# wangxb29/PPST

Measured on AMD Instinct MI355X. Metric: 512x512 portrait swaps/sec/GPU, higher is better.
Workload: dtype bf16x3 (fp32 split into hi+lo bf16, 3 MFMA passes, fp32 accumulate); 1 GPU; simple_swapping 512x512 batch=8 per GPU, generator+encoders forward only (BASELINE configs[1]); image_parallel=1 batch per rank, no data-path collective

## Files before the change

### include/ppst_hip.h

```cpp
#ifndef PPST_HIP_H
#define PPST_HIP_H

#include <stddef.h>
#include <stdint.h>

#ifdef __cplusplus
extern "C" {
#endif

#define PPST_OK 0
#define PPST_EINVAL (-1)
#define PPST_EUNSUPPORTED (-2)
#define PPST_ENULL (-3)

enum { PPST_F32 = 0, PPST_F16 = 1, PPST_BF16 = 2, PPST_F64 = 3  };

enum { PPST_PAD_ZERO = 0, PPST_PAD_REFLECT = 1, PPST_PAD_REPLICATE = 2 };

enum { PPST_ACT_NONE = 0, PPST_ACT_LRELU = 1 , PPST_ACT_PRELU = 2 };

#define PPST_ABI_VERSION 3
int ppst_version(void);

#define PPST_ST_F32 0
// ... 87 lines not shown
  int32_t out_h, out_w, out_ld, cout;
  int32_t nsteps, n_groups;
  int32_t pad_mode;
  int32_t in_off_y, in_off_x;
  int32_t out_sy, out_sx;
  int32_t act;
  int32_t precision;
  int32_t res_ld;
  int32_t tile_h, tile_w;
  int32_t halo;
  int32_t bn;
  const void* in_scale_shift;
  const void* in_prelu;
  int32_t in_c, in_act;
  int32_t flop_steps;
  int32_t tile_rows;
  int32_t a_slots;
  int32_t early_a;
  int32_t variant;
  int32_t reserved0;
  int32_t dual_b;
  int32_t io_st;
  int32_t k64;
  const void* in_res;
  int32_t in_res_ld;
  int32_t ksplit;
  const int32_t* ksplit_starts;
  void* ksplit_scratch;
  unsigned* ksplit_flags;
  uint32_t ksplit_epoch;
} ppst_conv_args;

int ppst_conv2d_mfma(const ppst_conv_args* a, void* stream);
int64_t ppst_conv_pack_wino_bytes(int cout, int cin);
int ppst_conv_pack_wino(const void* w, int64_t sn, int64_t sc, int64_t sy, int64_t sx, float scale, int cout, int cin,
                        void* out, void* stream);
int ppst_conv2d_f32(const ppst_conv_args* a, const void* w, int64_t sn, int64_t sc, int64_t sy, int64_t sx, float wscale,
                    const int32_t* src_c, const int32_t* src_ky, const int32_t* src_kx, void* stream);
int ppst_conv_tiles(int tile_h, int tile_w, int tile_rows);

int ppst_conv1x1_small_cin(const void* x, const void* w, const void* bias, void* y,
                           int64_t npix, int cin, int in_ld, int cout, float wscale,
                           int act, void* stream);
int ppst_conv1x1_small_cin_st(const void* x, const void* w, const void* bias, void* y,
                              int64_t npix, int cin, int in_ld, int cout, float wscale,
                              int act, int y_st , void* stream);
int ppst_conv1x1_small_cout(const void* x, const void* w, const void* bias, void* y,
                            int64_t npix, int cin, int cout, float wscale, void* stream);
int ppst_conv1x1_small_cout_st(const void* x, const void* w, const void* bias, void* y,
                               int64_t npix, int cin, int cout, float wscale, int x_st , void* stream);
int ppst_torgb_apply_st(const void* x, const void* scale_shift, const void* res, int res_ld, float out_scale, const void* w,
                        const void* bias, void* y, int B, int H, int W, int cin, float wscale, int x_st, void* stream);

int ppst_in_stats(const void* x, void* partial, int B, int H, int W, int C, int ld,
                  int rep_pad, int* n_partials, void* stream);
int ppst_in_finalize(const void* partial, int n_partials, const void* style,
                     int style_ld ,
                     const void* post_bias ,
                     void* scale_shift , int B, int C, double count,
                     float eps, void* stream);
int ppst_affine_act(const void* x, const void* scale_shift, const void* res,
                    const void* res_scale_shift , void* y,
                    int B, int64_t hw, int C, int x_ld, int res_ld, int y_ld,
                    int act , const void* prelu,
                    float out_scale,
                    int res_up2_w ,
// ... 328 lines not shown
```

### ppst_amd/_lib.py

```python
import ctypes
import os

import torch

HERE = os.path.dirname(os.path.abspath(__file__))
LIB_PATH = os.environ.get("PPST_HIP_LIB") or os.path.join(HERE, "libppst_hip.so")

if not os.path.exists(LIB_PATH):
    raise ImportError(
        "ppst_amd: %s is missing -- build it with `python -m ppst_amd.build` "
        "(hipcc --offload-arch=gfx950). There is no CPU fallback." % LIB_PATH)

lib = ctypes.CDLL(LIB_PATH)

vp, i32, i64, f32, f64 = ctypes.c_void_p, ctypes.c_int, ctypes.c_int64, ctypes.c_float, ctypes.c_double


class PackJob(ctypes.Structure):
    _fields_ = [("w", vp), ("sn", i64), ("sc", i64), ("sy", i64), ("sx", i64), ("src_c", vp), ("src_ky", vp), ("src_kx", vp),
                ("out", vp), ("total", i64), ("block0", i64), ("scale", f32), ("cout", i32), ("bn", i32), ("nsteps", i32),
                ("n_groups", i32), ("x3", i32), ("f16", i32), ("nblocks", i32), ("dual", i32)]


class UpscaleJob(ctypes.Structure):
# ... 47 lines not shown
        ("nsteps", i32), ("n_groups", i32), ("pad_mode", i32),
        ("in_off_y", i32), ("in_off_x", i32), ("out_sy", i32), ("out_sx", i32),
        ("act", i32), ("precision", i32), ("res_ld", i32), ("tile_h", i32), ("tile_w", i32),
        ("halo", i32), ("bn", i32), ("in_scale_shift", vp), ("in_prelu", vp), ("in_c", i32), ("in_act", i32),
        ("flop_steps", i32), ("tile_rows", i32), ("a_slots", i32), ("early_a", i32), ("variant", i32), ("reserved0", i32), ("dual_b", i32), ("io_st", i32), ("k64", i32),
        ("in_res", vp), ("in_res_ld", i32), ("ksplit", i32), ("ksplit_starts", vp),
        ("ksplit_scratch", vp), ("ksplit_flags", vp), ("ksplit_epoch", ctypes.c_uint32),
    ]


_SIGS = {
    "ppst_version": (i32, []),
    "ppst_guided_filter_tune": (i32, [i32, i32]),
    "ppst_upfirdn2d": (i32, [vp, vp, vp] + [i32] * 14 + [i32, vp]),
    "ppst_blur_nhwc": (i32, [vp, vp, vp] + [i32] * 10 + [vp, i32, vp]),
    "ppst_blur_nhwc_st": (i32, [vp, vp, vp] + [i32] * 10 + [vp, i32, i32, vp]),
    "ppst_fused_bias_act": (i32, [vp, vp, vp, vp, i64, i32, i32, i32, i32, f32, f32, i32, vp]),
    "ppst_nchw_to_nhwc": (i32, [vp, vp, i32, i32, i32, i32, vp]),
    "ppst_nhwc_to_nchw": (i32, [vp, vp, i32, i32, i32, i32, vp]),
    "ppst_conv_pack": (i32, [vp, i64, i64, i64, i64, f32, i32, i32, vp, vp, vp, i32, i32, i32, vp, vp]),
    "ppst_conv_pack_k64": (i32, [vp, i64, i64, i64, i64, f32, i32, i32, vp, vp, vp, i32, i32, i32, i32, vp, vp]),
    "ppst_conv_pack_up9_bytes": (i64, [i32, i32]),
    "ppst_conv_pack_up9": (i32, [vp, i64, i64, i64, i64, f32, i32, i32, vp, vp]),
    "ppst_conv_pack_wino_bytes": (i64, [i32, i32]),
    "ppst_conv_pack_wino": (i32, [vp, i64, i64, i64, i64, f32, i32, i32, vp, vp]),
    "ppst_conv_pack_dual": (i32, [vp, i64, i64, i64, i64, f32, i32, vp, vp, vp, i32, i32, i32, vp, vp]),
    "ppst_upscale_weight": (i32, [vp, vp, i32, i32, f32, vp]),
    "ppst_dgrad_s2d_stack_weight": (i32, [vp, vp, i32, i32, vp]),
    "ppst_depth_to_space_st": (i32, [vp, vp, i32, i32, i32, i32, i32, i32, i32, vp]),
    "ppst_pack_job_blocks": (i32, [i64]),
    "ppst_conv_pack_batch": (i32, [vp, i32, i32, vp]),
    "ppst_upscale_weight_batch": (i32, [vp, i32, i32, vp]),
    "ppst_conv2d_mfma": (i32, [ctypes.POINTER(ConvArgs), vp]),
    "ppst_conv2d_f32": (i32, [ctypes.POINTER(ConvArgs), vp, i64, i64, i64, i64, f32, vp, vp, vp, vp]),
    "ppst_conv_tiles": (i32, [i32, i32, i32]),
    "ppst_conv1x1_small_cin": (i32, [vp, vp, vp, vp, i64, i32, i32, i32, f32, i32, vp]),
    "ppst_conv1x1_small_cin_st": (i32, [vp, vp, vp, vp, i64, i32, i32, i32, f32, i32, i32, vp]),
    "ppst_conv1x1_small_cout": (i32, [vp, vp, vp, vp, i64, i32, i32, f32, vp]),
    "ppst_conv1x1_small_cout_st": (i32, [vp, vp, vp, vp, i64, i32, i32, f32, i32, vp]),
    "ppst_torgb_apply_st": (i32, [vp, vp, vp, i32, f32, vp, vp, vp, i32, i32, i32, i32, f32, i32, vp]),
    "ppst_in_stats": (i32, [vp, vp, i32, i32, i32, i32, i32, i32, ctypes.POINTER(i32), vp]),
    "ppst_in_finalize": (i32, [vp, i32, vp, i32, vp, vp, i32, i32, f64, f32, vp]),
    "ppst_affine_act": (i32, [vp, vp, vp, vp, vp, i32, i64, i32, i32, i32, i32, i32, vp, f32, i32, vp]),
    "ppst_affine_act_st": (i32, [vp, vp, vp, vp, vp, i32, i64, i32, i32, i32, i32, i32, vp, f32, i32, i32, i32, vp]),
    "ppst_affine_act_stats": (i32, [vp, vp, vp, vp, vp, vp, i32, i32, i32, i32, i32, i32, i32, i32, vp, f32, i32, i32, vp]),
    "ppst_upsample_nearest2": (i32, [vp, vp, i32, i32, i32, i32, vp]),
    "ppst_upsample_nearest2_st": (i32, [vp, vp, i32, i32, i32, i32, i32, vp]),
    "ppst_gap_gmp_ws": (i64, [i32, i64, i32]),
    "ppst_gap_gmp": (i32, [vp, vp, vp, vp, i32, i32, i32, i32, i32, vp]),
    "ppst_gap_gmp_st": (i32, [vp, vp, vp, vp, i32, i32, i32, i32, i32, i32, vp]),
    "ppst_avgpool": (i32, [vp, vp, i32, i32, i32, i32, i32, i32, i32, vp]),
    "ppst_bilinear": (i32, [vp, vp, i32, i32, i32, i32, i32, i32, i32, i32, vp]),
    "ppst_head_tail": (i32, [vp, vp, vp, vp, vp] + [i32] * 10 + [vp]),
    "ppst_maxpool2": (i32, [vp, vp, i32, i32, i32, i32, vp]),
    "ppst_linear": (i32, [vp, vp, vp, vp, i32, i32, i32, f32, f32, i32, i32, vp]),
    "ppst_l2norm_rows": (i32, [vp, vp, i32, i32, f32, i32, vp]),
    "ppst_lerp": (i32, [vp, vp, vp, i64, f32, vp]),
    "ppst_linear_grouped": (i32, [vp, i32, vp]),
    "ppst_l2norm_rows_grouped": (i32, [vp, i32, vp]),
    "ppst_lerp_grouped": (i32, [vp, i32, vp]),
    "ppst_gap_gmp_multi_level_ws": (i64, [vp, i32, i32]),
    "ppst_gap_gmp_multi_level": (i32, [vp, i32, i32, vp, i32, vp]),
    "ppst_spatial_modulation": (i32, [vp, vp, vp, vp, i32, i64, i32, vp]),
    "ppst_spatial_modulation_st": (i32, [vp, vp, vp, vp, i32, i64, i32, i32, vp]),
    "ppst_rselfcorr": (i32, [vp, vp, i32, i32, i32, i32, i32, vp]),
    "ppst_corr_prep": (i32, [vp, vp, i32, i32, i32, i32, vp]),
# ... 150 lines not shown
```

### ppst_amd/csrc/conv1x1.hip

```cpp
#include "conv_common.h"

struct C1Args {
  const float* x;
  const unsigned char* wpack;
  const int4* steps;
  float* y;
  const float* bias;
  const float* noise;
  const float* prelu;
  float* stats;
  const float* residual;
  float noise_weight, out_scale;
  int B, hw, in_ld, out_ld, cout, nsteps, act, res_ld, n_tiles, tiles;
  int in_h, in_w, out_h, out_w, tiles_x, pad_mode;
  const float* in_ss;
  const float* in_prelu;
  int in_c, in_act;
  const float* in_res;
  int in_res_ld;
};

#define C1_GROUP 8
#define C1_BLOB 8192

// ... 91 lines not shown
  };
  CONV_EPI_DISPATCH(SPEC, epi_passes, act, resm);
  if (a.stats) {
#pragma unroll
    for (int nt = 0; nt < NT; ++nt) {
      float4 u = s1[nt], w = s2[nt];
      float* uv[8] = {&u.x, &u.y, &u.z, &u.w, &w.x, &w.y, &w.z, &w.w};
#pragma unroll
      for (int q = 0; q < 8; ++q) {
        float t = *uv[q];
        t += __builtin_bit_cast(float, __builtin_amdgcn_mov_dpp(__builtin_bit_cast(int, t), 0xB1, 0xf, 0xf, true));
        t += __builtin_bit_cast(float, __builtin_amdgcn_mov_dpp(__builtin_bit_cast(int, t), 0x4E, 0xf, 0xf, true));
        t += __builtin_bit_cast(float, __builtin_amdgcn_mov_dpp(__builtin_bit_cast(int, t), 0x141, 0xf, 0xf, true));
        t += __builtin_bit_cast(float, __builtin_amdgcn_mov_dpp(__builtin_bit_cast(int, t), 0x140, 0xf, 0xf, true));
        *uv[q] = t;
      }
      if (r16 == 0) conv_epi_put_sums(&red[wave][nt * 16 + g * 4][0], u, w);
    }
    __syncthreads();
    if (tid < (NT > 4 ? 128 : 64)) {
      const int n = ntile * (NT > 4 ? 128 : 64) + tid;
      if (n < a.cout) {
        float t0 = 0.f, t1 = 0.f;
#pragma unroll
        for (int wv = 0; wv < 8; ++wv) { t0 += red[wv][tid][0]; t1 += red[wv][tid][1]; }
        float* o = a.stats + (((int64_t)b * a.tiles + mblk) * a.cout + n) * 2;
        o[0] = t0;
        o[1] = t1;
      }
    }
  }
}

template <int INSS, bool TAPS = false, int NT_ = 4, int PREC = 0, int IOS = PPST_ST_F32>
__global__ __launch_bounds__(512, 4) void conv1x1_stream_kernel(C1Args a) {
  constexpr int MT = 2, NT = NT_;
  constexpr bool X3 = PREC == 0;
  static_assert(IOS == PPST_ST_F32 || IOS == (PREC == 3 ? PPST_ST_F16 : PREC == 1 ? PPST_ST_BF16 : -1), "half storage: single-pass modes");
  constexpr int ES = IOS == PPST_ST_F32 ? 4 : 2;
  constexpr int BLOB1 = X3 ? C1_BLOB : C1_BLOB / 2;
  __shared__ uint4 sB[C1_GROUP * BLOB1 / 16];
  __shared__ float red[8][64][2];

  const int wid = xcd_block_id(blockIdx.x, gridDim.x);
  const int ntile = wid % a.n_tiles;
  int mblk = wid / a.n_tiles;
  const int b = mblk / a.tiles;
  mblk -= b * a.tiles;
  const int tid = threadIdx.x, lane = tid & 63, wave = __builtin_amdgcn_readfirstlane(tid >> 6);
  const int r16 = lane & 15, g = lane >> 4;
  const int pbase = mblk * 256 + wave * 32;
  const int tyi = TAPS ? mblk / a.tiles_x : 0, txi = TAPS ? mblk - tyi * a.tiles_x : 0;
  const int oy0 = tyi * 16 + wave * 2, ox = txi * 16 + r16;
  const unsigned char* xb = (const unsigned char*)a.x + (int64_t)b * (TAPS ? a.in_h * a.in_w : a.hw) * a.in_ld * ES;
  const unsigned char* wblob = a.wpack + (int64_t)ntile * a.nsteps * BLOB1;
#if defined(__HIP_DEVICE_COMPILE__)
  typedef const __attribute__((address_space(4))) int4* StepPtr;
#else
  typedef const int4* StepPtr;
#endif
  StepPtr steps = (StepPtr)a.steps;

  int64_t aoff[MT];
  bool pok[MT];
#pragma unroll
  for (int mt = 0; mt < MT; ++mt) {
    const int p = pbase + mt * 16 + r16;
    pok[mt] = TAPS ? true : p < a.hw;
    aoff[mt] = TAPS ? 0 : (int64_t)(pok[mt] ? p : 0) * a.in_ld + g * 8;
  }
  const float in_slope = (INSS && a.in_act == PPST_ACT_PRELU && a.in_prelu) ? a.in_prelu[0] : 0.f;
  auto in_act = [&](float t) -> float { return conv_in_act(t, a.in_act, in_slope); };

  f32x4 acc[MT][NT];
#pragma unroll
  for (int i = 0; i < MT; ++i)
#pragma unroll
    for (int j = 0; j < NT; ++j) acc[i][j] = (f32x4){0.f, 0.f, 0.f, 0.f};

  float4 raw[MT][2], ss[4];
  float4 rres[INSS == 2 ? MT : 1][2];
  auto a_load = [&](int4 d) {
    const int chan = d.x;
// ... 1 lines not shown
      int ix = ox + d.z;
      bool xok = ix >= 0 && ix < a.in_w;
      ix = conv_pad_index(ix, a.in_w, a.pad_mode);
#pragma unroll
      for (int mt = 0; mt < MT; ++mt) {
        int iy = oy0 + mt + d.y;
        const bool yok = iy >= 0 && iy < a.in_h;
        iy = conv_pad_index(iy, a.in_h, a.pad_mode);
        pok[mt] = a.pad_mode != PPST_PAD_ZERO || (xok && yok);
        aoff[mt] = ((int64_t)iy * a.in_w + ix) * a.in_ld + g * 8;
      }
    }
#pragma unroll
    for (int mt = 0; mt < MT; ++mt) {
      const float4* p = (const float4*)(xb + (aoff[mt] + chan) * ES);
      raw[mt][0] = p[0];
      if (IOS == PPST_ST_F32) raw[mt][1] = p[1];
      if (INSS == 2) {
        const int pp = pbase + mt * 16 + r16;
        const float4* q = (const float4*)(a.in_res + ((int64_t)b * a.hw + (pok[mt] ? pp : 0)) * a.in_res_ld + g * 8 + chan);
        rres[mt][0] = q[0];
        rres[mt][1] = q[1];
      }
    }
    if (INSS) {
      const float4* q = (const float4*)(a.in_ss + ((int64_t)b * a.in_c + chan + g * 8) * 2);
      ss[0] = q[0]; ss[1] = q[1]; ss[2] = q[2]; ss[3] = q[3];
    }
  };
  a_load(steps[0]);

  for (int s0 = 0; s0 < a.nsteps; s0 += C1_GROUP) {
    const int ng = a.nsteps - s0 < C1_GROUP ? a.nsteps - s0 : C1_GROUP;
    if (s0) __syncthreads();
    for (int i = tid; i < ng * (BLOB1 / 16); i += 512) sB[i] = ((const uint4*)(wblob + (int64_t)s0 * BLOB1))[i];
    __syncthreads();
    for (int sl = 0; sl < ng; ++sl) {
      const int s = s0 + sl;
      bf16x8 ah[MT], al[MT];
      bool vok[MT];
#pragma unroll
      for (int mt = 0; mt < MT; ++mt) vok[mt] = pok[mt];
#pragma unroll
      for (int mt = 0; mt < MT; ++mt) {
        if (IOS != PPST_ST_F32 && !INSS) {
          const float4 z = vok[mt] ? raw[mt][0] : make_float4(0.f, 0.f, 0.f, 0.f);
          ah[mt] = __builtin_bit_cast(bf16x8, z);
          al[mt] = ah[mt];
          continue;
        }
        float v[8] = {raw[mt][0].x, raw[mt][0].y, raw[mt][0].z, raw[mt][0].w, raw[mt][1].x, raw[mt][1].y, raw[mt][1].z, raw[mt][1].w};
        if (IOS != PPST_ST_F32) c1_unpack8<IOS>(raw[mt][0], v);
        if (INSS) {
          const float sc[8] = {ss[0].x, ss[0].z, ss[1].x, ss[1].z, ss[2].x, ss[2].z, ss[3].x, ss[3].z};
          const float sh[8] = {ss[0].y, ss[0].w, ss[1].y, ss[1].w, ss[2].y, ss[2].w, ss[3].y, ss[3].w};
#pragma unroll
          for (int j = 0; j < 8; ++j) {
            float t = sc[j] * v[j] + sh[j];
            if (INSS == 2) {
              const float4 r4 = rres[mt][j >> 2];
              t += (j & 3) == 0 ? r4.x : (j & 3) == 1 ? r4.y : (j & 3) == 2 ? r4.z : r4.w;
            }
            v[j] = in_act(t);
          }
        }
#pragma unroll
        for (int j = 0; j < 8; ++j)
          if (!vok[mt]) v[j] = 0.f;
        c1_cvt8<PREC>(v, ah[mt], al[mt]);
      }
      if (s + 1 < a.nsteps) a_load(steps[s + 1]);
      const unsigned char* bs = (const unsigned char*)sB + sl * BLOB1 + g * 1024 + r16 * 16;
#pragma unroll
      for (int nt = 0; nt < NT; ++nt) {
        const bf16x8 bh = *(const bf16x8*)(bs + nt * 256);
        bf16x8 bl = bh;
        if (X3) bl = *(const bf16x8*)(bs + nt * 256 + 4096);
#pragma unroll
        for (int mt = 0; mt < MT; ++mt) acc[mt][nt] = c1_mfma<PREC>(bh, bl, ah[mt], al[mt], acc[mt][nt]);
      }
    }
  }

  c1_epilogue<MT, NT, TAPS, X3, IOS>(a, acc, red, b, mblk, ntile, pbase, oy0, ox, tid, wave, r16, g);
}

#define C3_GROUP 9
template <int CTRL>
__device__ __forceinline__ bf16x8 c3_shift(bf16x8 edge, bf16x8 centre) {
  typedef int __attribute__((ext_vector_type(4))) i4;
  const i4 e = __builtin_bit_cast(i4, edge), c = __builtin_bit_cast(i4, centre);
  i4 r;
#pragma unroll
  for (int i = 0; i < 4; ++i) r[i] = __builtin_amdgcn_update_dpp(e[i], c[i], CTRL, 0xf, 0xf, false);
  return __builtin_bit_cast(bf16x8, r);
}

template <bool INSS, int NT_, int PREC = 0, int IOS = PPST_ST_F32>
__global__ __launch_bounds__(512, NT_ > 4 ? 2 : 4) void conv3x3_direct_kernel(C1Args a) {
  constexpr int MT = 2, NT = NT_;
  constexpr bool X3 = PREC == 0;
  static_assert(IOS == PPST_ST_F32 || IOS == (PREC == 3 ? PPST_ST_F16 : PREC == 1 ? PPST_ST_BF16 : -1), "half storage: single-pass modes");
  constexpr int ES = IOS == PPST_ST_F32 ? 4 : 2;
  constexpr int PSTR = (NT > 4 ? 128 : 64) * 16;
  constexpr int BLOB = (X3 ? 8 : 4) * PSTR;
  __shared__ uint4 sB[C3_GROUP * BLOB / 16];
  __shared__ float red[8][NT > 4 ? 128 : 64][2];
  const int tid = threadIdx.x, lane = tid & 63, wave = __builtin_amdgcn_readfirstlane(tid >> 6);
  const int r16 = lane & 15, g = lane >> 4;
  const int total = a.B * a.tiles * a.n_tiles;
  const int per = (total + (int)gridDim.x - 1) / (int)gridDim.x;
  const int w_beg = blockIdx.x * per, w_end = w_beg + per < total ? w_beg + per : total;
  const int nchunks = a.nsteps / 9;
  const bool keep_b = nchunks == 1 && a.n_tiles == 1;
  for (int wid = w_beg; wid < w_end; ++wid) {
  const int ntile = wid % a.n_tiles;
  int mblk = wid / a.n_tiles;
// ... 75 lines not shown
#pragma unroll
    for (int r = 0; r < 4; ++r) {
      bf16x8 ch, cl, eh, el;
      convert(rawc, okc, ch, cl);
      convert(rawe, oke, eh, el);
      if (r < 3) row_load(chan, r + 1);
      else if (c + 1 < nchunks) { ss_load(chan_next); row_load(chan_next, 0); }
#pragma unroll
      for (int dxi = 0; dxi < 3; ++dxi) {
        const bf16x8 fh = dxi == 0 ? c3_shift<0x111>(eh, ch) : (dxi == 1 ? ch : c3_shift<0x101>(eh, ch));
        const bf16x8 fl = dxi == 0 ? c3_shift<0x111>(el, cl) : (dxi == 1 ? cl : c3_shift<0x101>(el, cl));
#pragma unroll
        for (int mt = 0; mt < MT; ++mt) {
          const int dyi = r - mt;
          if (dyi < 0 || dyi > 2) continue;
          const unsigned char* bs = (const unsigned char*)sB + (dyi * 3 + dxi) * BLOB + g * PSTR + r16 * 16;
#pragma unroll
          for (int nt = 0; nt < NT; ++nt) {
            const bf16x8 bh = *(const bf16x8*)(bs + nt * 256);
            bf16x8 bl = bh;
            if (X3) bl = *(const bf16x8*)(bs + nt * 256 + 4 * PSTR);
            acc[mt][nt] = c1_mfma<PREC>(bh, bl, fh, fl, acc[mt][nt]);
          }
        }
        __builtin_amdgcn_sched_barrier(0);
      }
    }
    chan = chan_next;
  }
  c1_epilogue<MT, NT, true, (X3 && NT <= 4), IOS>(a, acc, red, b, mblk, ntile, 0, oy0, ox, tid, wave, r16, g);
  }
}

static inline int64_t blocks_of(const ppst_conv_args* a, int tiles, int n_tiles) { return (int64_t)a->B * tiles * n_tiles; }
int ppst_conv1x1_stream_launch(const ppst_conv_args* a, int n_tiles, int tiles, hipStream_t st) {
  C1Args k;
  k.x = (const float*)a->x; k.wpack = (const unsigned char*)a->wpack; k.steps = (const int4*)a->steps; k.y = (float*)a->y;
  k.bias = (const float*)a->bias; k.noise = (const float*)a->noise; k.prelu = (const float*)a->prelu;
  k.stats = (float*)a->stats; k.residual = (const float*)a->residual;
  k.noise_weight = a->noise_weight; k.out_scale = a->out_scale;
  k.B = a->B; k.hw = a->out_h * a->out_w; k.in_ld = a->in_ld; k.out_ld = a->out_ld; k.cout = a->cout; k.nsteps = a->nsteps;
  k.act = a->act; k.res_ld = a->res_ld; k.n_tiles = n_tiles; k.tiles = tiles;
  k.in_ss = (const float*)a->in_scale_shift; k.in_prelu = (const float*)a->in_prelu; k.in_c = a->in_c; k.in_act = a->in_act;
  k.in_res = (const float*)a->in_res; k.in_res_ld = a->in_res_ld;
  if ((int64_t)tiles * 256 < k.hw) return PPST_EINVAL;
  if (k.in_res) {
    PPST_LAUNCH((conv1x1_stream_kernel<2, false, 4, 0, PPST_ST_F32>), dim3((unsigned)blocks_of(a, tiles, n_tiles)), dim3(512), 0, st, k);
    return PPST_LAUNCH_CHECK();
  }
  const int64_t blocks = (int64_t)a->B * tiles * n_tiles;
  if (blocks > 0x7fffffff) return PPST_EINVAL;
#define LS(PREC_, IOS_)                                                                                               \
  do {                                                                                                                \
    if (k.in_ss) PPST_LAUNCH((conv1x1_stream_kernel<1, false, 4, PREC_, IOS_>), dim3((unsigned)blocks), dim3(512), 0, st, k);   \
    else PPST_LAUNCH((conv1x1_stream_kernel<0, false, 4, PREC_, IOS_>), dim3((unsigned)blocks), dim3(512), 0, st, k);          \
  } while (0)
  if (a->precision == 1) { if (a->io_st) LS(1, PPST_ST_BF16); else LS(1, PPST_ST_F32); }
  else if (a->precision == 3) { if (a->io_st) LS(3, PPST_ST_F16); else LS(3, PPST_ST_F32); }
  else LS(0, PPST_ST_F32);
#undef LS
  return PPST_LAUNCH_CHECK();
}

int ppst_conv_direct_launch(const ppst_conv_args* a, int n_tiles, int tiles_y, int tiles_x, hipStream_t st) {
  C1Args k;
  k.x = (const float*)a->x; k.wpack = (const unsigned char*)a->wpack; k.steps = (const int4*)a->steps; k.y = (float*)a->y;
  k.bias = (const float*)a->bias; k.noise = (const float*)a->noise; k.prelu = (const float*)a->prelu;
  k.stats = (float*)a->stats; k.residual = (const float*)a->residual;
  k.noise_weight = a->noise_weight; k.out_scale = a->out_scale;
  k.B = a->B; k.hw = a->out_h * a->out_w; k.in_ld = a->in_ld; k.out_ld = a->out_ld; k.cout = a->cout; k.nsteps = a->nsteps;
  k.act = a->act; k.res_ld = a->res_ld; k.n_tiles = n_tiles; k.tiles = tiles_y * tiles_x;
  k.in_ss = (const float*)a->in_scale_shift; k.in_prelu = (const float*)a->in_prelu; k.in_c = a->in_c; k.in_act = a->in_act;
  k.in_h = a->in_h; k.in_w = a->in_w; k.out_h = a->out_h; k.out_w = a->out_w; k.tiles_x = tiles_x; k.pad_mode = a->pad_mode;
  const int64_t blocks = (int64_t)a->B * k.tiles * n_tiles;
  if (blocks > 0x7fffffff) return PPST_EINVAL;
  const bool nt2 = a->cout <= 32;
#define LD(INSS_, PREC_, IOS_)                                                                                       \
  do {                                                                                                               \
    if (nt2) PPST_LAUNCH((conv1x1_stream_kernel<INSS_, true, 2, PREC_, IOS_>), dim3((unsigned)blocks), dim3(512), 0, st, k);       \
    else PPST_LAUNCH((conv1x1_stream_kernel<INSS_, true, 4, PREC_, IOS_>), dim3((unsigned)blocks), dim3(512), 0, st, k);           \
  } while (0)
#define LDP(PREC_, IOS_) do { if (k.in_ss) LD(1, PREC_, IOS_); else LD(0, PREC_, IOS_); } while (0)
  if (a->precision == 1) { if (a->io_st) LDP(1, PPST_ST_BF16); else LDP(1, PPST_ST_F32); }
  else if (a->precision == 3) { if (a->io_st) LDP(3, PPST_ST_F16); else LDP(3, PPST_ST_F32); }
  else LDP(0, PPST_ST_F32);
#undef LDP
#undef LD
  return PPST_LAUNCH_CHECK();
}

int ppst_conv3x3_direct_launch(const ppst_conv_args* a, int n_tiles, int tiles_y, int tiles_x, hipStream_t st) {
  if (a->nsteps % 9) return PPST_EINVAL;
  C1Args k;
// ... 28 lines not shown
```

### ppst_amd/csrc/conv_mfma.hip

```cpp
#include "conv_common.h"


#ifdef PPST_CONV_CLOCK
__device__ unsigned long long* g_clock_buf = nullptr;
__device__ int g_clock_n = 1;
extern "C" int ppst_conv_clock_buffer(void* buf, int n) {
  if (n <= 0) return PPST_EINVAL;
  if (hipMemcpyToSymbol(HIP_SYMBOL(g_clock_buf), &buf, sizeof(buf)) != hipSuccess) return PPST_EINVAL;
  return hipMemcpyToSymbol(HIP_SYMBOL(g_clock_n), &n, sizeof(n)) == hipSuccess ? PPST_OK : PPST_EINVAL;
}
#endif
typedef _Float16 __attribute__((ext_vector_type(8))) half8;
__device__ __forceinline__ unsigned short f2h(float f) { return __builtin_bit_cast(unsigned short, (_Float16)f); }
template <int WM, int WN, int HALO, bool X3, bool INSS, int NAS = 0, bool F16 = false, int IOS = PPST_ST_F32>
__global__ __launch_bounds__(64 * WM * WN, NAS ? 2 : 1) void conv_mfma_kernel(ConvKArgs a) {
  static_assert(IOS == PPST_ST_F32 || (!X3 && IOS == (F16 ? PPST_ST_F16 : PPST_ST_BF16)), "half storage: single-pass modes");
  constexpr int ES = IOS == PPST_ST_F32 ? 4 : 2;
  constexpr int NT = 64 * WM * WN;
  constexpr int TH = 4 * WM, TW = 16;
  constexpr int HH = TH + 2 * HALO, HW = TW + 2 * HALO, HP = HH * HW;
  constexpr int PLANE = (WM == 2) ? HP * 16 : ((HP * 16 + 255) / 256) * 256;
  constexpr int NPL = X3 ? 8 : 4;
  constexpr int NPLB = X3 ? 8 : 4;
  constexpr int ABUF = NPL * PLANE;
// ... 621 lines not shown
extern "C" int ppst_prof_enable(int on) {
  g_prof_on = on;
  g_ev_used = 0;
  if (on) g_prof_dropped = 0;
  return PPST_OK;
}
extern "C" int ppst_prof_collect(double* ms, int64_t* launches, double* flop) {
  double t = 0.0, f = 0.0;
  for (int i = 0; i < g_ev_used; ++i) {
    float e = 0.f;
    hipError_t err = hipEventElapsedTime(&e, g_ev[i][0], g_ev[i][1]);
    if (err != hipSuccess) return (int)err;
    t += e;
    f += g_flop[i];
  }
  if (ms) *ms = t;
  if (launches) *launches = g_ev_used;
  if (flop) *flop = f;
  g_ev_used = 0;
  return PPST_OK;
}
extern "C" int ppst_prof_detail(int idx, double* ms, double* flop, int32_t* info) {
  if (idx < 0 || idx >= g_ev_used) return PPST_EINVAL;
  float e = 0.f;
  hipError_t err = hipEventElapsedTime(&e, g_ev[idx][0], g_ev[idx][1]);
  if (err != hipSuccess) return (int)err;
  if (ms) *ms = e;
  if (flop) *flop = g_flop[idx];
  if (info) for (int i = 0; i < 8; ++i) info[i] = g_info[idx][i];
  return PPST_OK;
}

int ppst_conv2d_mfma2_launch(const ppst_conv_args* a, int n_tiles, int tiles_y, int tiles_x, hipStream_t st);
int ppst_conv1x1_stream_launch(const ppst_conv_args* a, int n_tiles, int tiles, hipStream_t st);
int ppst_conv_direct_launch(const ppst_conv_args* a, int n_tiles, int tiles_y, int tiles_x, hipStream_t st);
int ppst_conv3x3_direct_launch(const ppst_conv_args* a, int n_tiles, int tiles_y, int tiles_x, hipStream_t st);
int ppst_conv_wino_launch(const ppst_conv_args* a, int n_tiles, int tiles_y, int tiles_x, hipStream_t st);

int ppst_ksplit_prepare_(const ppst_conv_args* a, int64_t tiles, int acc_regs, int threads, KSplitDev* out) {
  const int S = a->ksplit, nsteps = a->nsteps;
  const int32_t* starts = a->ksplit_starts;
  if ((S != 2 && S != 4 && S != 8) || (!starts && nsteps % S) || tiles <= 0 || acc_regs <= 0 || acc_regs % 4 || threads <= 0) return PPST_EINVAL;
  if (S == 8 && acc_regs > 64) return PPST_EINVAL;
  for (int i = 0; i <= S; ++i) {
    out->start[i] = starts ? starts[i] : i * (nsteps / S);
    if (i && out->start[i] <= out->start[i - 1]) return PPST_EINVAL;
  }
  if (out->start[0] != 0 || out->start[S] != nsteps) return PPST_EINVAL;
  const int64_t slots = (int64_t)(S - 1) * tiles;
  if (slots > KS_MAX_SLOTS || slots > PPST_KSPLIT_FLAG_WORDS - 1 || (size_t)slots * threads * acc_regs * 4 > PPST_KSPLIT_SCRATCH_BYTES) return PPST_EINVAL;
  if (!a->ksplit_scratch || !a->ksplit_flags) return PPST_ENULL;
  if (a->ksplit_epoch == 0) return PPST_EINVAL;
  out->scratch = (float*)a->ksplit_scratch; out->flags = a->ksplit_flags; out->epoch = a->ksplit_epoch; out->S = S;
  return PPST_OK;
}

extern "C" int ppst_conv_tiles(int tile_h, int tile_w, int tile_rows) { return cdiv(tile_h, tile_rows) * cdiv(tile_w, tile_rows == 15 ? 15 : 16); }

template <int WM, int WN, int HALO, bool X3, int NAS = 0, bool F16 = false, int IOS = PPST_ST_F32>
static void launch_conv(const ConvKArgs& k, int blocks, hipStream_t st) {
  const dim3 grid(blocks, k.ks.S > 1 ? k.ks.S : 1);
  if (k.in_ss) PPST_LAUNCH((conv_mfma_kernel<WM, WN, HALO, X3, true, NAS, F16, IOS>), grid, dim3(64 * WM * WN), 0, st, k);
  else PPST_LAUNCH((conv_mfma_kernel<WM, WN, HALO, X3, false, NAS, F16, IOS>), grid, dim3(64 * WM * WN), 0, st, k);
}

extern "C" int ppst_conv2d_mfma(const ppst_conv_args* a, void* stream) {
  if (!a) return PPST_ENULL;
  if (a->B < 0 || a->in_h <= 0 || a->in_w <= 0 || a->in_ld <= 0 || a->in_ld % 4 || a->out_h <= 0 || a->out_w <= 0 ||
      a->out_ld < a->cout || a->cout <= 0 || a->cout % 4 || a->out_ld % 4 || (a->residual && a->res_ld % 4) || a->nsteps <= 0 ||
      (a->n_groups != 1 && a->n_groups != 4 && !(a->n_groups == 2 && a->dual_b)) || a->pad_mode < 0 ||
      (a->dual_b && (a->variant != 2 || a->bn != 256 || a->n_groups != 2 || a->halo != 1 || (a->precision != 0 && a->precision != 1 && a->precision != 3) || a->out_sy != 2 || a->out_sx != 2 || !a->early_a)) ||
      a->pad_mode > 2 || a->tile_h <= 0 || a->tile_w <= 0 || a->out_sy <= 0 || a->out_sx <= 0 ||
      (a->precision != 0 && a->precision != 1 && a->precision != 3) || a->halo < 0 || a->halo > 1 || (a->bn != 64 && a->bn != 128 && a->bn != 256) || (a->residual && a->res_ld < a->cout) ||
      a->variant < 0 || a->variant > 11 || (a->variant == 0 && a->bn == 256) ||
      (a->variant == 11 && (a->precision != 0 || a->bn != 256 || a->halo != 1 || a->n_groups != 1 || a->out_sy != 2 || a->out_sx != 2 ||
                            !a->early_a || a->tile_rows != 15 || a->pad_mode != PPST_PAD_ZERO || a->in_scale_shift || a->residual ||
                            (a->act & 0xff) == PPST_ACT_PRELU || a->cout % 64 || a->nsteps % 4 || a->in_off_y || a->in_off_x ||
                            a->tile_h != a->in_h || a->tile_w != a->in_w || a->out_h != 2 * a->in_h || a->out_w != 2 * a->in_w || a->io_st)) ||
      (a->variant == 10 && (a->precision != 0 || a->bn != 128 || a->halo != 1 || a->n_groups != 1 || a->out_sy != 1 || a->out_sx != 1 ||
                            a->in_off_y != 0 || a->in_off_x != 0 || a->tile_h != a->out_h || a->tile_w != a->out_w ||
                            a->in_h != a->out_h || a->in_w != a->out_w || a->nsteps % 9 != 0 || a->tile_rows != 16 ||
                            (a->in_scale_shift && a->nsteps / 9 > 32))) ||
      ((a->variant == 2 || a->variant == 7 || a->variant == 9) &&
       ((a->precision != 0 && !((a->variant == 2 || a->variant == 7 || (a->variant == 9 && a->k64)) && (a->precision == 1 || a->precision == 3))) || a->bn == 64 || !a->early_a)) ||
      (a->variant == 7 && (a->bn != 128 || a->tile_rows != 32)) ||
      (a->variant == 9 && (a->bn != 128 || a->tile_rows != 24)) ||
      (a->variant == 2 && a->bn != 256) ||
      (a->variant == 4 && ((a->precision != 0 && a->precision != 1 && a->precision != 3) || a->bn != 64 || a->halo != 0 || a->n_groups != 1 || a->out_sy != 1 || a->out_sx != 1 ||
                           a->in_off_y != 0 || a->in_off_x != 0 || a->tile_h != a->out_h || a->tile_w != a->out_w ||
                           a->in_h != a->out_h || a->in_w != a->out_w)) ||
      (a->in_res && (a->variant != 4 || !a->in_scale_shift || a->precision != 0 || a->io_st || a->in_res_ld < a->in_c || a->in_res_ld % 4 ||
                     ((uintptr_t)a->in_res % 16))) ||
      ((a->variant == 5 || a->variant == 6) && ((a->precision != 0 && a->precision != 1 && a->precision != 3) ||
                                                (a->bn != 64 && !(a->variant == 6 && a->bn == 128 && a->precision == 0)) || a->n_groups != 1 || a->out_sy != 1 || a->out_sx != 1 ||
                           a->in_off_y != 0 || a->in_off_x != 0 || a->tile_h != a->out_h || a->tile_w != a->out_w)) ||
      (a->tile_rows != 16 && !(a->variant == 7 && a->tile_rows == 32) && !(a->variant == 9 && a->tile_rows == 24) && !(a->variant == 11 && a->tile_rows == 15) &&
       !(a->variant == 0 && a->tile_rows == 8 && a->bn == 128 && a->halo == 1 && a->early_a && a->precision == 0)) || (a->in_scale_shift && a->in_c <= 0) || a->a_slots < 0 || a->a_slots > 3)
    return PPST_EINVAL;
  if (a->variant == 1 || a->variant == 3 || (a->variant == 7 && a->precision == 0) || a->variant == 8 || (a->variant == 9 && !a->k64) ||
// ... 7 lines not shown
    return PPST_EINVAL;
  {
    const int64_t px = (int64_t)a->out_h * a->out_w + 64 * (int64_t)a->out_sx;
    if (px * a->out_ld > 0x7fffffff || (a->residual && px * a->res_ld > 0x7fffffff)) return PPST_EINVAL;
  }
  if ((int64_t)a->in_h * a->in_w * a->in_ld * 4 > 0x7fffffff) return PPST_EINVAL;
  if (a->io_st && (((uintptr_t)a->x | (uintptr_t)a->y | (uintptr_t)a->residual) % 8)) return PPST_EINVAL;
  if (a->io_st && a->variant >= 4 && a->variant <= 6 && (a->in_ld % 8 || (uintptr_t)a->x % 16)) return PPST_EINVAL;
  if ((a->tile_h - 1) * a->out_sy >= a->out_h || (a->tile_w - 1) * a->out_sx >= a->out_w) return PPST_EINVAL;
  if (a->B == 0) return PPST_OK;
  if (!a->x || !a->wpack || !a->steps || !a->y) return PPST_ENULL;
  ConvKArgs k = conv_kargs_fill(a, cdiv(a->cout, a->variant == 11 ? 64 : a->dual_b ? a->bn / 2 : a->bn), cdiv(a->tile_h, a->tile_rows),
                                cdiv(a->tile_w, a->variant == 11 ? 15 : 16));
  int64_t blocks64 = (int64_t)a->n_groups * k.n_tiles * a->B * k.tiles_y * k.tiles_x;
  if (blocks64 > 0x7fffffff) return PPST_EINVAL;
  int blocks = (int)blocks64;
  hipStream_t st = as_stream(stream);
  if (a->ksplit > 1) {
    if (a->variant == 0) {
      if (a->tile_rows != 16 && a->tile_rows != 8) return PPST_EINVAL;
      const int e0 = ppst_ksplit_prepare_(a, blocks, 64, (a->bn == 128 && a->tile_rows == 16) ? 512 : 256, &k.ks);
      if (e0 != PPST_OK) return e0;
    } else if (a->variant != 2 && a->variant != 10) return PPST_EINVAL;
  }
  k.prefetch_w = (int64_t)blocks * k.ks.S <= 512 ? 1 : 0;
  int slot = -1;
  if (g_prof_on) {
    const int inf[8] = {a->B, a->tile_h, a->tile_w, a->nsteps, a->cout, a->n_groups, a->halo,
                        a->bn | (a->variant << 12) | ((a->k64 ? 1 : 0) << 20) | (a->precision << 24)};
    slot = ppst_prof_begin_(2.0 * 32.0 * (a->flop_steps > 0 ? a->flop_steps : a->nsteps) * (double)((a->dual_b || a->variant == 11) ? 4 : a->n_groups) * a->cout * (double)a->B * a->tile_h * a->tile_w,
                            inf, st);
  }
  if (a->variant >= 1) {
    int e2 = a->variant == 4   ? ppst_conv1x1_stream_launch(a, k.n_tiles, k.tiles_y * k.tiles_x, st)
             : a->variant == 5 ? ppst_conv_direct_launch(a, k.n_tiles, k.tiles_y, k.tiles_x, st)
             : a->variant == 6 ? ppst_conv3x3_direct_launch(a, k.n_tiles, k.tiles_y, k.tiles_x, st)
             : a->variant == 10 ? ppst_conv_wino_launch(a, k.n_tiles, k.tiles_y, k.tiles_x, st)
                               : ppst_conv2d_mfma2_launch(a, k.n_tiles, k.tiles_y, k.tiles_x, st);
    if (slot >= 0) (void)hipEventRecord(g_ev[slot][1], st);
    return e2;
  }
  const bool x3 = a->precision == 0;
  const bool f16 = a->precision == 3, hs = a->io_st != 0;
#define DISPATCH(WM_, WN_)                                                                                         \
  do {                                                                                                             \
    if (a->halo) { if (x3) launch_conv<WM_, WN_, 1, true>(k, blocks, st); else if (f16 && hs) launch_conv<WM_, WN_, 1, false, 0, true, PPST_ST_F16>(k, blocks, st); else if (f16) launch_conv<WM_, WN_, 1, false, 0, true>(k, blocks, st); else if (hs) launch_conv<WM_, WN_, 1, false, 0, false, PPST_ST_BF16>(k, blocks, st); else launch_conv<WM_, WN_, 1, false>(k, blocks, st); } \
    else         { if (x3) launch_conv<WM_, WN_, 0, true>(k, blocks, st); else if (f16 && hs) launch_conv<WM_, WN_, 0, false, 0, true, PPST_ST_F16>(k, blocks, st); else if (f16) launch_conv<WM_, WN_, 0, false, 0, true>(k, blocks, st); else if (hs) launch_conv<WM_, WN_, 0, false, 0, false, PPST_ST_BF16>(k, blocks, st); else launch_conv<WM_, WN_, 0, false>(k, blocks, st); } \
  } while (0)
  if (a->tile_rows == 8) launch_conv<2, 2, 1, true, 2>(k, blocks, st);
  else if (a->bn == 64 && x3 && a->halo == 1 && a->a_slots == 1) launch_conv<4, 1, 1, true, 1>(k, blocks, st);
  else if (a->bn == 64 && x3 && a->halo == 0 && a->a_slots == 1) launch_conv<4, 1, 0, true, 1>(k, blocks, st);
  else if (a->bn == 64 && x3 && a->halo == 0 && a->a_slots == 2) launch_conv<4, 1, 0, true, 2>(k, blocks, st);
  else if (a->bn == 128) DISPATCH(4, 2); else DISPATCH(4, 1);
#undef DISPATCH
  int e = PPST_LAUNCH_CHECK();
  if (slot >= 0) (void)hipEventRecord(g_ev[slot][1], st);
  return e;
}
```

### ppst_amd/ops.py

```python
import collections
import ctypes
import os
import threading
import types

import torch

from . import _lib, conv_tables
from ._lib import lib, check

PAD_ZERO, PAD_REFLECT, PAD_REPLICATE = 0, 1, 2
ACT_NONE, ACT_LRELU, ACT_PRELU = 0, 1, 2
RES_BEFORE_ACT = 1 << 8

PRECISION = {"value": 0}
TILE_ROWS = {"value": 16}
CONV_VARIANT = {"value": 2}
DUAL_CONVT = {"value": True, "min_blocks": 32}
UP9 = {"value": True, "min_blocks": 64, "min_fill": 0.85}
DIRECT_MAX = {"cout": 64, "nsteps": 40, "cout3x3": 64}
WGRAD_SPLIT = {"blocks": 1024, "min_tiles": 4}
WGRAD_TR2_BLOCKS = 512
WGRAD_TR2_MIN_TILES = 8
STREAM_1X1 = {"value": True}
# ... 352 lines not shown
            elif single:
                if (self.bn == 128 and self.halo == 1 and self.n_groups == 1 and TALL_TILE_SINGLE["value"] and
                        _tiles(th, tw, 32) * ((self.cout + 127) // 128) >= TALL_TILE_SINGLE["min_blocks"]):
                    variant, rows = 7, 32
            elif (self.bn == 128 and self.halo == 1 and (small or (TWO_BLOCK_8ROW["value"] and
                  _tiles(th, tw, 8) * self.n_groups * ((self.cout + 127) // 128) >= TWO_BLOCK_8ROW["min_blocks"]))):
                rows = 8
        same = (th, tw) == (oh, ow)
        if STREAM_1X1["value"] and self.halo == 0 and self.n_groups == 1 and osy == 1 and same and (oh, ow) == (H, W):
            variant, bn, rows = 4, 64, TILE_ROWS["value"]
        elif (self.halo == 1 and self.n_groups == 1 and osy == 1 and same and self.cout <= DIRECT_MAX["cout"]
              and self.nsteps <= DIRECT_MAX["nsteps"]):
            variant, bn, rows = (6 if (self.kind in ("conv", "dgrad") and self.k == 3) else 5), 64, TILE_ROWS["value"]
        elif (not single and self.kind in ("conv", "dgrad") and self.k == 3 and 64 < self.cout <= DIRECT_MAX["cout3x3"] and same):
            variant, bn, rows = 6, 128, TILE_ROWS["value"]
        return variant, bn, rows

    def _ksplit(self, variant, a, skip):
        if (skip or variant not in KSPLIT["variants"]
                or not (a.tile_rows == 16 or (variant == 0 and a.tile_rows == 8))):
            return 0, None
        cs = self.chunk_starts0_k64 if a.k64 else self.chunk_starts0
        if cs is None or cs[-1] != a.nsteps:
            return 0, None
        if a.dual_b or (variant == 2 and ((self.precision == 0) != (a.io_st == 0) or (a.k64 and not a.halo))):
            return 0, None
        n_tiles = -(-self.cout // a.bn)
        blocks = a.B * lib.ppst_conv_tiles(a.tile_h, a.tile_w, a.tile_rows) * a.n_groups * n_tiles
        max_s, min_steps = {0: (8, KSPLIT["min_steps"]), 2: (4, 24), 10: (2, 36)}[variant]
        return _ksplit_choice(blocks, cs, KSPLIT["max_blocks"], min_steps, max_s)

    def __call__(self, x, bias=None, noise=None, noise_weight=0.0, act=ACT_NONE, prelu=None, stats=False,
                 residual=None, out=None, out_scale=1.0, pad_mode=PAD_ZERO, out_hw=None, res_after_act=False,
                 in_ss=None, in_act=ACT_NONE, in_prelu=None, in_res=None):
        in_ld = _nhwc_ld(x, "conv input", half_ok=True)
        B, H, W, xc = x.shape
        if x.dtype != torch.float32 and {torch.float16: 3, torch.bfloat16: 1}[x.dtype] != self.precision:
            raise RuntimeError("conv input stored as %s needs a plan of the matching single-pass precision mode (plan: mode %d)"
                               % (x.dtype, self.precision))
        need_c = self.max_chan + 32
        if xc < need_c:
            raise RuntimeError("conv input has %d channels (pixel stride %d); the %s plan reads %d" % (xc, in_ld, self.kind, need_c))
        if in_ss is not None and (in_ss.dim() != 3 or in_ss.shape[0] != B or in_ss.shape[1] < need_c or in_ss.shape[2] != 2
                                  or not in_ss.is_contiguous()):
            raise RuntimeError("in_ss must be a contiguous (B=%d, >=%d, 2) table, got %s" % (B, need_c, tuple(in_ss.shape)))
        if self.kind == "convT":
            th, tw, oh, ow, osy = H, W, 2 * H, 2 * W, 2
        elif self.kind == "dgrad_s2d":
            oh, ow = out_hw
            th, tw, osy = (oh + 1) // 2, (ow + 1) // 2, 2
        elif self.kind in ("s2d", "dgrad_s2ds"):
            oh, ow = out_hw
            th, tw, osy = oh, ow, 1
        else:
            th, tw, oh, ow, osy = H, W, H, W, 1
        if out is None:
            out = torch.empty((B, oh, ow, self.cout), device=x.device, dtype=x.dtype)
        out_ld = _nhwc_ld(out, "conv output", half_ok=True)
        if out.dtype != x.dtype or (residual is not None and residual.dtype != x.dtype):
            raise RuntimeError("conv input, residual and output share one storage type (ppst_conv_args.io_st): got %s / %s / %s"
                               % (x.dtype, None if residual is None else residual.dtype, out.dtype))
        if tuple(out.shape) != (B, oh, ow, self.cout):
            raise RuntimeError("conv output must be %s, got %s" % ((B, oh, ow, self.cout), tuple(out.shape)))
        if noise is not None and (noise.numel() != B * oh * ow or not noise.is_contiguous()):
            raise RuntimeError("noise must be a contiguous (B,1,%d,%d) tensor with B = %d rows, got %s" % (oh, ow, B, tuple(noise.shape)))
        if residual is not None and tuple(residual.shape) != (B, oh, ow, self.cout):
            raise RuntimeError("residual must match the output shape %s, got %s" % ((B, oh, ow, self.cout), tuple(residual.shape)))
# ... 21 lines not shown
        a.res_ld = _nhwc_ld(residual, "residual", half_ok=True) if residual is not None else 0
        a.io_st = _ST[x.dtype]
        a.noise_weight, a.out_scale = float(noise_weight), float(out_scale)
        a.B, a.in_h, a.in_w, a.in_ld = B, H, W, in_ld
        a.out_h, a.out_w, a.out_ld, a.cout = oh, ow, out_ld, self.cout
        a.nsteps, a.n_groups, a.pad_mode = form.nsteps, form.n_groups, pad_mode
        a.in_off_y = a.in_off_x = 0
        a.out_sy = a.out_sx = osy
        a.act, a.precision = act | (0x100 if res_after_act else 0), self.precision
        a.tile_h, a.tile_w, a.halo, a.bn, a.tile_rows = th, tw, self.halo, bn, rows
        _chk(in_ss, "in_ss"); _chk(in_prelu, "in_prelu")
        a.in_scale_shift, a.in_prelu, a.in_act = _p(in_ss), _p(in_prelu), in_act
        a.in_c = in_ss.shape[1] if in_ss is not None else 0
        if in_res is not None:
            if variant != 4 or in_ss is None or self.precision != 0 or x.dtype != torch.float32:
                raise RuntimeError("in_res needs a 1x1 plan on the streaming kernel (ops.STREAM_1X1), in_ss, precision 0 and fp32 storage")
            if tuple(in_res.shape) != tuple(x.shape):
                raise RuntimeError("in_res must have the conv input's shape %s, got %s" % (tuple(x.shape), tuple(in_res.shape)))
            a.in_res, a.in_res_ld = _p(in_res), _nhwc_ld(in_res, "in_res")
        a.flop_steps = self.flop_steps
        a.a_slots = min(3, self.chunks_per_group)
        a.early_a = self.early_a
        ks_S, ks_cuts = self._ksplit(variant, a, self.precision == 2) if (KSPLIT["value"] and BATCH_AWARE["value"]) else (0, None)
        stream = _stream()
        if ks_S:
            ks_arr = (ctypes.c_int32 * (ks_S + 1))(*ks_cuts)
            a.ksplit, a.ksplit_starts = ks_S, ctypes.cast(ks_arr, ctypes.c_void_p)
            a.ksplit_scratch, a.ksplit_flags, a.ksplit_epoch = _ksplit_next(stream)
        if self.precision == 2:
            sn, sc, sy, sx = self.wstrides
            c_, ky_, kx_ = self.src_dev
            check(lib.ppst_conv2d_f32(ctypes.byref(a), _p(self.wsrc), sn, sc, sy, sx, self.scale, _p(c_), _p(ky_), _p(kx_), stream),
                  "ppst_conv2d_f32")
        else:
            check(lib.ppst_conv2d_mfma(ctypes.byref(a), stream), "ppst_conv2d_mfma")
        if stats:
            return out, st
        return out


class _KsWorkspace:
    __slots__ = ("scratch", "flags", "ptrs", "launches")

    def __init__(self):
        self.scratch = torch.empty(KSPLIT_SCRATCH_BYTES, dtype=torch.uint8, device="cuda")
        self.flags = torch.zeros(KSPLIT_FLAG_WORDS, dtype=torch.int32, device="cuda")
        self.ptrs = self.scratch.data_ptr(), self.flags.data_ptr()
        self.launches = 0


_ks_ws = {}
_ks_lock = threading.Lock()


def _ks_key(stream):
    return (_cur_device() if _cur_device is not None else torch.cuda.current_device()), stream.value


def _ksplit_next(stream):
    key = _ks_key(stream)
    with _ks_lock:
        ws = _ks_ws.get(key)
        if ws is None:
            ws = _ks_ws[key] = _KsWorkspace()
        ws.launches += 1
        epoch = (ws.launches - 1) % 0xFFFFFFFF + 1
# ... 1591 lines not shown
```

Measured before the change: 162.8 swaps/s (all GPUs).

## Add persistent-block mode to 1x1 streaming conv kernel with weight-tile reuse

```diff
diff --git a/include/ppst_hip.h b/include/ppst_hip.h
--- a/include/ppst_hip.h
+++ b/include/ppst_hip.h
@@ -143,6 +143,7 @@
 } ppst_conv_args;
 
 int ppst_conv2d_mfma(const ppst_conv_args* a, void* stream);
+int ppst_conv1x1_stream(const ppst_conv_args* a, int max_blocks, void* stream);
 int64_t ppst_conv_pack_wino_bytes(int cout, int cin);
 int ppst_conv_pack_wino(const void* w, int64_t sn, int64_t sc, int64_t sy, int64_t sx, float scale, int cout, int cin,
                         void* out, void* stream);
diff --git a/ppst_amd/_lib.py b/ppst_amd/_lib.py
--- a/ppst_amd/_lib.py
+++ b/ppst_amd/_lib.py
@@ -103,6 +103,7 @@
     "ppst_conv_pack_batch": (i32, [vp, i32, i32, vp]),
     "ppst_upscale_weight_batch": (i32, [vp, i32, i32, vp]),
     "ppst_conv2d_mfma": (i32, [ctypes.POINTER(ConvArgs), vp]),
+    "ppst_conv1x1_stream": (i32, [ctypes.POINTER(ConvArgs), i32, vp]),
     "ppst_conv2d_f32": (i32, [ctypes.POINTER(ConvArgs), vp, i64, i64, i64, i64, f32, vp, vp, vp, vp]),
     "ppst_conv_tiles": (i32, [i32, i32, i32]),
     "ppst_conv1x1_small_cin": (i32, [vp, vp, vp, vp, i64, i32, i32, i32, f32, i32, vp]),
diff --git a/ppst_amd/csrc/conv1x1.hip b/ppst_amd/csrc/conv1x1.hip
--- a/ppst_amd/csrc/conv1x1.hip
+++ b/ppst_amd/csrc/conv1x1.hip
@@ -147,23 +147,27 @@
   }
 }
 
-template <int INSS, bool TAPS = false, int NT_ = 4, int PREC = 0, int IOS = PPST_ST_F32>
+template <int INSS, bool TAPS = false, int NT_ = 4, int PREC = 0, int IOS = PPST_ST_F32, bool PERS = false>
 __global__ __launch_bounds__(512, 4) void conv1x1_stream_kernel(C1Args a) {
+  static_assert(!PERS || (!TAPS && INSS != 2), "persistent blocks: the plain and normalise-on-load 1x1 instances");
   constexpr int MT = 2, NT = NT_;
   constexpr bool X3 = PREC == 0;
   static_assert(IOS == PPST_ST_F32 || IOS == (PREC == 3 ? PPST_ST_F16 : PREC == 1 ? PPST_ST_BF16 : -1), "half storage: single-pass modes");
   constexpr int ES = IOS == PPST_ST_F32 ? 4 : 2;
   constexpr int BLOB1 = X3 ? C1_BLOB : C1_BLOB / 2;
   __shared__ uint4 sB[C1_GROUP * BLOB1 / 16];
-  __shared__ float red[8][64][2];
-
-  const int wid = xcd_block_id(blockIdx.x, gridDim.x);
+  __shared__ float red[PERS ? 2 : 1][8][64][2];
+
+  const int tid = threadIdx.x, lane = tid & 63, wave = __builtin_amdgcn_readfirstlane(tid >> 6);
+  const int r16 = lane & 15, g = lane >> 4;
+  const int wid0 = xcd_block_id(blockIdx.x, gridDim.x);
+  const int w_end = PERS ? a.B * a.tiles * a.n_tiles : wid0 + 1, w_step = PERS ? (int)gridDim.x : 1;
+  int sb_ntile = -1, par = 0;
+  for (int wid = wid0; wid < w_end; wid += w_step) {
   const int ntile = wid % a.n_tiles;
   int mblk = wid / a.n_tiles;
   const int b = mblk / a.tiles;
   mblk -= b * a.tiles;
-  const int tid = threadIdx.x, lane = tid & 63, wave = __builtin_amdgcn_readfirstlane(tid >> 6);
-  const int r16 = lane & 15, g = lane >> 4;
   const int pbase = mblk * 256 + wave * 32;
   const int tyi = TAPS ? mblk / a.tiles_x : 0, txi = TAPS ? mblk - tyi * a.tiles_x : 0;
   const int oy0 = tyi * 16 + wave * 2, ox = txi * 16 + r16;
@@ -231,9 +235,11 @@
 
   for (int s0 = 0; s0 < a.nsteps; s0 += C1_GROUP) {
     const int ng = a.nsteps - s0 < C1_GROUP ? a.nsteps - s0 : C1_GROUP;
-    if (s0) __syncthreads();
-    for (int i = tid; i < ng * (BLOB1 / 16); i += 512) sB[i] = ((const uint4*)(wblob + (int64_t)s0 * BLOB1))[i];
-    __syncthreads();
+    if (!PERS || a.nsteps > C1_GROUP || sb_ntile != ntile) {
+      if (s0 || wid != wid0) __syncthreads();
+      for (int i = tid; i < ng * (BLOB1 / 16); i += 512) sB[i] = ((const uint4*)(wblob + (int64_t)s0 * BLOB1))[i];
+      __syncthreads();
+    }
     for (int sl = 0; sl < ng; ++sl) {
       const int s = s0 + sl;
       bf16x8 ah[MT], al[MT];
@@ -281,7 +287,9 @@
     }
   }
 
-  c1_epilogue<MT, NT, TAPS, X3, IOS>(a, acc, red, b, mblk, ntile, pbase, oy0, ox, tid, wave, r16, g);
+  c1_epilogue<MT, NT, TAPS, X3, IOS>(a, acc, red[par], b, mblk, ntile, pbase, oy0, ox, tid, wave, r16, g);
+  if (PERS) { sb_ntile = ntile; par ^= 1; }
+  }
 }
 
 #define C3_GROUP 9
@@ -423,8 +431,8 @@
   }
 }
 
-static inline int64_t blocks_of(const ppst_conv_args* a, int tiles, int n_tiles) { return (int64_t)a->B * tiles * n_tiles; }
-int ppst_conv1x1_stream_launch(const ppst_conv_args* a, int n_tiles, int tiles, hipStream_t st) {
+#define C1_RESIDENT 512
+int ppst_conv1x1_stream_launch(const ppst_conv_args* a, int n_tiles, int tiles, int max_blocks, hipStream_t st) {
   C1Args k;
   k.x = (const float*)a->x; k.wpack = (const unsigned char*)a->wpack; k.steps = (const int4*)a->steps; k.y = (float*)a->y;
   k.bias = (const float*)a->bias; k.noise = (const float*)a->noise; k.prelu = (const float*)a->prelu;
@@ -434,22 +442,28 @@
   k.act = a->act; k.res_ld = a->res_ld; k.n_tiles = n_tiles; k.tiles = tiles;
   k.in_ss = (const float*)a->in_scale_shift; k.in_prelu = (const float*)a->in_prelu; k.in_c = a->in_c; k.in_act = a->in_act;
   k.in_res = (const float*)a->in_res; k.in_res_ld = a->in_res_ld;
-  if ((int64_t)tiles * 256 < k.hw) return PPST_EINVAL;
+  if ((int64_t)tiles * 256 < k.hw || max_blocks < 0) return PPST_EINVAL;
+  const int64_t total = (int64_t)a->B * tiles * n_tiles;
+  if (total > 0x7fffffff) return PPST_EINVAL;
   if (k.in_res) {
-    PPST_LAUNCH((conv1x1_stream_kernel<2, false, 4, 0, PPST_ST_F32>), dim3((unsigned)blocks_of(a, tiles, n_tiles)), dim3(512), 0, st, k);
+    PPST_LAUNCH((conv1x1_stream_kernel<2, false, 4, 0, PPST_ST_F32>), dim3((unsigned)total), dim3(512), 0, st, k);
     return PPST_LAUNCH_CHECK();
   }
-  const int64_t blocks = (int64_t)a->B * tiles * n_tiles;
-  if (blocks > 0x7fffffff) return PPST_EINVAL;
-#define LS(PREC_, IOS_)                                                                                               \
+  int cap = max_blocks ? max_blocks : C1_RESIDENT;
+  if (cap >= n_tiles) cap -= cap % n_tiles;
+  const bool pers = total <= (1 << 30) && (max_blocks || (a->nsteps >= 4 && total > cap));
+  const int64_t blocks = pers && cap < total ? cap : total;
+#define LS2(INSS_, PREC_, IOS_)                                                                                        \
   do {                                                                                                                \
-    if (k.in_ss) PPST_LAUNCH((conv1x1_stream_kernel<1, false, 4, PREC_, IOS_>), dim3((unsigned)blocks), dim3(512), 0, st, k);   \
-    else PPST_LAUNCH((conv1x1_stream_kernel<0, false, 4, PREC_, IOS_>), dim3((unsigned)blocks), dim3(512), 0, st, k);          \
+    if (pers) PPST_LAUNCH((conv1x1_stream_kernel<INSS_, false, 4, PREC_, IOS_, true>), dim3((unsigned)blocks), dim3(512), 0, st, k);   \
+    else PPST_LAUNCH((conv1x1_stream_kernel<INSS_, false, 4, PREC_, IOS_, false>), dim3((unsigned)blocks), dim3(512), 0, st, k);       \
   } while (0)
+#define LS(PREC_, IOS_) do { if (k.in_ss) LS2(1, PREC_, IOS_); else LS2(0, PREC_, IOS_); } while (0)
   if (a->precision == 1) { if (a->io_st) LS(1, PPST_ST_BF16); else LS(1, PPST_ST_F32); }
   else if (a->precision == 3) { if (a->io_st) LS(3, PPST_ST_F16); else LS(3, PPST_ST_F32); }
   else LS(0, PPST_ST_F32);
 #undef LS
+#undef LS2
   return PPST_LAUNCH_CHECK();
 }
 
diff --git a/ppst_amd/csrc/conv_mfma.hip b/ppst_amd/csrc/conv_mfma.hip
--- a/ppst_amd/csrc/conv_mfma.hip
+++ b/ppst_amd/csrc/conv_mfma.hip
@@ -677,7 +677,7 @@
 }
 
 int ppst_conv2d_mfma2_launch(const ppst_conv_args* a, int n_tiles, int tiles_y, int tiles_x, hipStream_t st);
-int ppst_conv1x1_stream_launch(const ppst_conv_args* a, int n_tiles, int tiles, hipStream_t st);
+int ppst_conv1x1_stream_launch(const ppst_conv_args* a, int n_tiles, int tiles, int max_blocks, hipStream_t st);
 int ppst_conv_direct_launch(const ppst_conv_args* a, int n_tiles, int tiles_y, int tiles_x, hipStream_t st);
 int ppst_conv3x3_direct_launch(const ppst_conv_args* a, int n_tiles, int tiles_y, int tiles_x, hipStream_t st);
 int ppst_conv_wino_launch(const ppst_conv_args* a, int n_tiles, int tiles_y, int tiles_x, hipStream_t st);
@@ -709,7 +709,7 @@
   else PPST_LAUNCH((conv_mfma_kernel<WM, WN, HALO, X3, false, NAS, F16, IOS>), grid, dim3(64 * WM * WN), 0, st, k);
 }
 
-extern "C" int ppst_conv2d_mfma(const ppst_conv_args* a, void* stream) {
+static int conv2d_mfma_run(const ppst_conv_args* a, void* stream, int c1_max_blocks) {
   if (!a) return PPST_ENULL;
   if (a->B < 0 || a->in_h <= 0 || a->in_w <= 0 || a->in_ld <= 0 || a->in_ld % 4 || a->out_h <= 0 || a->out_w <= 0 ||
       a->out_ld < a->cout || a->cout <= 0 || a->cout % 4 || a->out_ld % 4 || (a->residual && a->res_ld % 4) || a->nsteps <= 0 ||
@@ -783,7 +783,7 @@
                             inf, st);
   }
   if (a->variant >= 1) {
-    int e2 = a->variant == 4   ? ppst_conv1x1_stream_launch(a, k.n_tiles, k.tiles_y * k.tiles_x, st)
+    int e2 = a->variant == 4   ? ppst_conv1x1_stream_launch(a, k.n_tiles, k.tiles_y * k.tiles_x, c1_max_blocks, st)
              : a->variant == 5 ? ppst_conv_direct_launch(a, k.n_tiles, k.tiles_y, k.tiles_x, st)
              : a->variant == 6 ? ppst_conv3x3_direct_launch(a, k.n_tiles, k.tiles_y, k.tiles_x, st)
              : a->variant == 10 ? ppst_conv_wino_launch(a, k.n_tiles, k.tiles_y, k.tiles_x, st)
@@ -808,3 +808,11 @@
   if (slot >= 0) (void)hipEventRecord(g_ev[slot][1], st);
   return e;
 }
+
+extern "C" int ppst_conv2d_mfma(const ppst_conv_args* a, void* stream) { return conv2d_mfma_run(a, stream, 0); }
+
+extern "C" int ppst_conv1x1_stream(const ppst_conv_args* a, int max_blocks, void* stream) {
+  if (!a) return PPST_ENULL;
+  if (a->variant != 4 || max_blocks < 0) return PPST_EINVAL;
+  return conv2d_mfma_run(a, stream, max_blocks);
+}
diff --git a/ppst_amd/ops.py b/ppst_amd/ops.py
--- a/ppst_amd/ops.py
+++ b/ppst_amd/ops.py
@@ -408,7 +408,7 @@
 
     def __call__(self, x, bias=None, noise=None, noise_weight=0.0, act=ACT_NONE, prelu=None, stats=False,
                  residual=None, out=None, out_scale=1.0, pad_mode=PAD_ZERO, out_hw=None, res_after_act=False,
-                 in_ss=None, in_act=ACT_NONE, in_prelu=None, in_res=None):
+                 in_ss=None, in_act=ACT_NONE, in_prelu=None, in_res=None, stream_max_blocks=None):
         in_ld = _nhwc_ld(x, "conv input", half_ok=True)
         B, H, W, xc = x.shape
         if x.dtype != torch.float32 and {torch.float16: 3, torch.bfloat16: 1}[x.dtype] != self.precision:
@@ -496,6 +496,10 @@
             c_, ky_, kx_ = self.src_dev
             check(lib.ppst_conv2d_f32(ctypes.byref(a), _p(self.wsrc), sn, sc, sy, sx, self.scale, _p(c_), _p(ky_), _p(kx_), stream),
                   "ppst_conv2d_f32")
+        elif stream_max_blocks is not None:
+            if variant != 4:
+                raise RuntimeError("stream_max_blocks needs a 1x1 plan on the streaming kernel (ops.STREAM_1X1)")
+            check(lib.ppst_conv1x1_stream(ctypes.byref(a), int(stream_max_blocks), stream), "ppst_conv1x1_stream")
         else:
             check(lib.ppst_conv2d_mfma(ctypes.byref(a), stream), "ppst_conv2d_mfma")
         if stats:
```

Measured after the change: 162.6 swaps/s (all GPUs). No clear change (-0.1%).
